# yifita/iso-points

Hardware: AMD Instinct MI355X
Metric: Mpoints/s full iso-point cycle (project+resample+splat), 1M pts (higher is better)
Workload: dtype f32-class (split-fp16 operands, 2^-22: hidden-layer products from two fp16 parts per f32 operand under exact power-of-two scales, 3 fp16-MFMA passes, f32 accumulate; everything else f32)

## Files before the change

iso_points_amd/csrc/bricks.hip:

```cpp
#include <type_traits>
#include "bricks.h"

#pragma clang fp contract(off)

constexpr int kScan1MaxWords = 2048;
BrickWs bricks_carve(void* ws, int64_t n_max) {
  BrickWs w;
  if (n_max < 1) n_max = 1;
  w.nb_cap = bricks_nb_cap(n_max);
  w.G = BK_CPB * (int64_t)w.nb_cap * w.nb_cap * w.nb_cap + 1;
  auto al = [](int64_t b) { return (b + 255) / 256 * 256; };
  char* p = (char*)ws;
  int64_t o = 0;
  w.hdr = (BrickHdr*)(p + o); o += al(sizeof(BrickHdr));
  w.counters = (int32_t*)(p + o); o += al(4 * kCounterInts);
  w.scan1 = (unsigned*)(p + o); o += al(4 * kScan1MaxWords);
  w.cnt = (int32_t*)(p + o); o += al(4 * w.G);
  w.off = (int32_t*)(p + o); o += al(4 * w.G);
  w.slot = (int32_t*)(p + o); o += al(4 * n_max);
  w.rec0 = (float4*)(p + o); o += al(16 * n_max);
  w.rec1 = (float4*)(p + o); o += al(16 * n_max);
  w.list = (int32_t*)(p + o); o += al(4 * (w.G < n_max ? w.G : n_max));
  w.tail = (int32_t*)(p + o); o += al(4 * 8 * n_max);
  w.scan_ws_bytes = iso_prefix_sum_workspace_bytes(w.G, 1) + 4 * (kScan1MaxWords + (w.G + 1023) / 1024);
// ... 984 lines not shown
__device__ __forceinline__ float wave_merge3(const Top3<KMAX>& best, int K, Emit&& emit) {
  int head = 0;
  float kth = FLT_MAX;
  for (int k = 0; k < K; ++k) {
    float hd = FLT_MAX;
    int hi = 0x7fffffff, ha = 0;
#pragma unroll
    for (int j = 0; j < KMAX; ++j) if (j == head) { hd = best.d[j]; hi = best.id[j]; ha = best.at[j]; }
    float md = hd;
    int mi = hi, ma = ha;
#pragma unroll
    for (int o = 32; o > 0; o >>= 1) {
      const float od = __shfl_xor(md, o);
      const int oi = __shfl_xor(mi, o), oa = __shfl_xor(ma, o);
      if (pair_lt(od, oi, md, mi)) { md = od; mi = oi; ma = oa; }
    }
    if (hd == md && hi == mi && md < FLT_MAX) ++head;
    if (k == K - 1) kth = md;
    emit(k, md, mi, ma);
  }
  return kth;
}

template <int KMAX>
__global__ __launch_bounds__(64) void k_brick_resample_tail(
    const BrickHdr* __restrict__ hp, const int32_t* __restrict__ off, const float4* __restrict__ rec0,
    const float4* __restrict__ rec1, const float* __restrict__ pts, int K, float* __restrict__ out,
    int64_t* __restrict__ idx_out, float* __restrict__ d2_out, const int32_t* __restrict__ tail,
    const int32_t* __restrict__ counters) {
  const BrickHdr h = *hp;
  const int lane = threadIdx.x;
  const int count = counters[1];
  const float B = 4.0f * h.f;
  const int rho_max = max(h.nb[0], max(h.nb[1], h.nb[2]));
  for (int w = blockIdx.x; w < count; w += gridDim.x) {
    const int row = tail[w];
    const float qx = pts[(int64_t)row * 3], qy = pts[(int64_t)row * 3 + 1], qz = pts[(int64_t)row * 3 + 2];
    const int qbx = bk_fine(qx, h.mn[0], h.inv_f, h.nf[0]) >> 2;
    const int qby = bk_fine(qy, h.mn[1], h.inv_f, h.nf[1]) >> 2;
    const int qbz = bk_fine(qz, h.mn[2], h.inv_f, h.nf[2]) >> 2;
    Top3<KMAX> best;
    best.init();
    float wd = FLT_MAX;
    int wi = 0x7fffffff;
    int found = 0;
    const WalkGeo geo = {qx, qy, qz, h.mn[0], h.mn[1], h.mn[2], B};
    float kth_seen = FLT_MAX;
    auto far2 = [&]() {
      float m = wd;
#pragma unroll
      for (int o = 32; o > 0; o >>= 1) m = fminf(m, __shfl_xor(m, o));
      return fminf(h.r2, fminf(m, kth_seen));
    };
    for (int rho = 0; rho <= rho_max; ++rho) {
      bk_walk_ring(rho, qbx, qby, qbz, h.nb[0], h.nb[1], h.nb[2], off, lane, geo, [&](int i) { return rec0[i]; },
                   [&](int i, const float4& c) {
        const float d2 = bk_d2(qx, qy, qz, c.x, c.y, c.z);
        if (d2 < h.r2) {
          if (found < KMAX) ++found;
          const int ci = __float_as_int(c.w);
          if (pair_lt(d2, ci, wd, wi)) {
            best.push(d2, ci, i, K);
#pragma unroll
            for (int j = 0; j < KMAX; ++j) if (j == K - 1) { wd = best.d[j]; wi = best.id[j]; }
          }
        }
      }, far2, far2);
      if (rho >= 1) {
        const float gg = (float)rho * B * 0.999f;
        if (gg >= h.r) break;
        int tot = found;
#pragma unroll
        for (int o = 32; o > 0; o >>= 1) tot += __shfl_xor(tot, o);
        if (tot >= K) {
          const float kth = wave_merge3<KMAX>(best, K, [](int, float, int, int) {});
          kth_seen = fminf(kth_seen, kth);
          if (kth < FLT_MAX && kth <= gg * gg) break;
        }
      }
    }
    Repulse R;
    R.px = qx; R.py = qy; R.pz = qz; R.inv_sigma = h.inv_sigma;
    const float kthf = wave_merge3<KMAX>(best, K, [&](int k, float md, int mi, int ma) {
      if (k == 0) return;
      if (md < FLT_MAX) {
        const float4 c = rec0[ma];
        const float4 u = rec1[ma];
        R.add(c.x, c.y, c.z, u.x, u.y, u.z);
      }
      if (idx_out && lane == 0) {
        idx_out[(int64_t)row * (K - 1) + k - 1] = md < FLT_MAX ? (int64_t)mi : (int64_t)-1;
        if (d2_out) d2_out[(int64_t)row * (K - 1) + k - 1] = md < FLT_MAX ? md : -1.0f;
      }
    });
    if (lane == 0) {
      R.finish(out + (int64_t)row * 3);
      const float need = kthf < FLT_MAX ? sqrtf(kthf) : h.r;
      if (qx - need < h.x_lo || qx + need >= h.x_hi) atomicAdd(const_cast<int32_t*>(&counters[6]), 1);
    }
  }
}

__global__ __launch_bounds__(256) void k_view_mask(const float* __restrict__ pts, const float* __restrict__ nrm,
                                                   const float* __restrict__ views, int n_views, int64_t n,
                                                   float znear, float zfar, int backface,
                                                   int32_t* __restrict__ mask, int32_t* __restrict__ view_count) {
  __shared__ int s_cnt[8];
  if (threadIdx.x < 8) s_cnt[threadIdx.x] = 0;
  __syncthreads();
  int local[8] = {0, 0, 0, 0, 0, 0, 0, 0};
  for (int64_t i = (int64_t)blockIdx.x * blockDim.x + threadIdx.x; i < n; i += (int64_t)gridDim.x * blockDim.x) {
    const float x = pts[i * 3], y = pts[i * 3 + 1], z = pts[i * 3 + 2];
    float nx = 0.f, ny = 0.f, nz = 0.f;
    if (backface) { nx = nrm[i * 3]; ny = nrm[i * 3 + 1]; nz = nrm[i * 3 + 2]; }
    int m = 0;
#pragma unroll
    for (int v = 0; v < 8; ++v) {
      if (v < n_views) {
        const float* V = views + v * 16;
        const float zv = ((x * V[2] + y * V[6]) + z * V[10]) + V[14];
// ... 197 lines not shown
  int pool_buf = 0;
  for (int w = blockIdx.x; w < count; w += gridDim.x) {
    const int row = tail[w] >> 3, v = tail[w] & 7;
    if (v >= n_views || !((mask[row] >> v) & 1)) continue;
    const float qx = pts[(int64_t)row * 3], qy = pts[(int64_t)row * 3 + 1], qz = pts[(int64_t)row * 3 + 2];
    const int qbx = bk_fine(qx, h.mn[0], h.inv_f, h.nf[0]) >> 2;
    const int qby = bk_fine(qy, h.mn[1], h.inv_f, h.nf[1]) >> 2;
    const int qbz = bk_fine(qz, h.mn[2], h.inv_f, h.nf[2]) >> 2;
    const bool small_cloud = view_total[v] < 7;
    TopF<7> best;
    best.init();
    float m7[7];
    const WalkGeo geo = {qx, qy, qz, h.mn[0], h.mn[1], h.mn[2], B};
    float kth_seen = FLT_MAX;
    bool sat = false;
    bool sat_any = false;
    bool sat_all = false;
    auto far2 = [&]() {
      float m = best.d[6];
#pragma unroll
      for (int o = 32; o > 0; o >>= 1) m = fminf(m, __shfl_xor(m, o));
      sat_any = sat_any || __any(sat);
      return fminf(sat_any ? kHSat : h.r2, fminf(m, kth_seen));
    };
    auto far2_all = [&]() { return fminf(sat_all ? kHSat : h.r2, kth_seen); };
    auto pool = [&]() {
      wave_merge_f7(best, m7);
      sat_any = sat_any || __any(sat);
      if (lane < 8) {
        float mine = m7[0];
#pragma unroll
        for (int k = 1; k < 7; ++k) mine = lane == k ? m7[k] : mine;
        s_m7[pool_buf][wave][lane] = lane == 7 ? (sat_any ? 1.f : 0.f) : mine;
      }
      __syncthreads();
      TopF<7> all;
      all.init();
      if (lane < 7 * kTailWaves) all.push(s_m7[pool_buf][lane / 7][lane % 7]);
      wave_merge_f7(all, m7);
#pragma unroll
      for (int k = 0; k < kTailWaves; ++k) sat_any = sat_any || s_m7[pool_buf][k][7] != 0.f;
      sat_all = sat_any;
      pool_buf ^= 1;
    };
    auto fetch = [&](int i) { float4 c = rec0[i]; c.w = rec1[i].w; return c; };
    auto visit = [&](int, const float4& c) {
      if (!((__float_as_int(c.w) >> v) & 1)) return;
      const float d2 = bk_d2(qx, qy, qz, c.x, c.y, c.z);
      if (d2 < kHSat) { if (d2 < h.r2) best.push(d2); }
      else if (d2 < h.r2) sat = true;
    };
    int rho_r = 1;
    while (rho_r < rho_max && (float)rho_r * B * 0.999f < h.r) ++rho_r;
    for (int rho = 0; rho <= min(1, rho_max); ++rho) {
      bk_walk_ring(rho, qbx, qby, qbz, h.nb[0], h.nb[1], h.nb[2], off, lane, geo, fetch, visit, far2_all, far2, wave, kTailWaves);
      if (rho >= 1) {
        const float gg = (float)rho * B * 0.999f;
        if (gg >= h.r) { rho_r = 1; break; }
        pool();
        kth_seen = fminf(kth_seen, m7[6]);
        if (m7[6] < FLT_MAX && m7[6] <= gg * gg) { rho_r = 1; break; }
        if (sat_any && kHSat <= gg * gg) { rho_r = 1; break; }
      }
    }
    if (rho_r > 1)
      bk_walk_shell(1, rho_r, qbx, qby, qbz, h.nb[0], h.nb[1], h.nb[2], off, lane, geo, fetch, visit, far2_all, far2, wave, kTailWaves);
    pool();
    if (threadIdx.x == 0) {
      const bool saturated = m7[6] == FLT_MAX && sat_any && !small_cloud;
      h_out[(int64_t)v * h.n_own + row] = saturated ? 0.01f : h_from_list(m7, small_cloud);
      const float need = m7[6] < FLT_MAX ? sqrtf(m7[6]) : (sat_any ? fminf(sqrtf(kHSat), h.r) : h.r);
      if (!small_cloud && (qx - need < h.x_lo || qx + need >= h.x_hi)) atomicAdd(const_cast<int32_t*>(&counters[6]), 1);
    }
  }
}

__device__ __forceinline__ void wave_append(bool take, int32_t* counter, int cap, int& slot) {
  const int lane = threadIdx.x & 63;
  const unsigned long long bal = __ballot(take);
  int base = 0;
  if (lane == 0 && bal) base = atomicAdd(counter, __popcll(bal));
  base = __shfl(base, 0);
  slot = take ? base + __popcll(bal & ((1ull << lane) - 1ull)) : -1;
  if (slot >= cap) slot = -1;
}

__global__ __launch_bounds__(256) void k_halo_export(const float* __restrict__ pts, const float* __restrict__ nrm,
                                                     const int32_t* __restrict__ payload, int64_t n_own,
                                                     const BrickHdr* __restrict__ hp, const float* __restrict__ ranges,
                                                     int world, int rank, int halo, float4* __restrict__ out, int cap) {
  const BrickHdr h = *hp;
  __shared__ int s_app[17];
  int32_t* counter = reinterpret_cast<int32_t*>(out);
  const int64_t span = (int64_t)gridDim.x * 1024;
  for (int64_t i0 = (int64_t)blockIdx.x * 1024; i0 < n_own; i0 += span) {
    bool take[4];
#pragma unroll
    for (int q = 0; q < 4; ++q) {
      const int64_t i = i0 + q * 256 + threadIdx.x;
      take[q] = false;
      if (i < n_own) {
        const int fx = bk_fine(pts[i * 3], h.mn[0], h.inv_f, h.nf[0]);
        for (int k = 0; k < world; ++k) {
          if (k == rank) continue;
          const int lo = bk_fine(ranges[k * 8], h.mn[0], h.inv_f, h.nf[0]) - halo;
          const int hi = bk_fine(ranges[k * 8 + 4], h.mn[0], h.inv_f, h.nf[0]) + halo;
          take[q] = take[q] || (fx >= lo && fx <= hi);
        }
      }
    }
    int slot[4];
    iso_block_append4(take, counter, s_app, slot);
#pragma unroll
    for (int q = 0; q < 4; ++q) {
      if (slot[q] >= 0 && slot[q] < cap) {
// ... 351 lines not shown
```

iso_points_amd/csrc/siren.hip:

```cpp
#include <stdlib.h>
#include "siren_common.h"
#include "iso_newton.h"
#include "mlp_common.h"

namespace {

__global__ void k_siren_pack(const float* __restrict__ raw, float* __restrict__ packed,
                             int H, int L) {
  const int64_t total = off_hidden(H, L);
  const int64_t HH = (int64_t)H * H;
  const int NT = H / 16;
  for (int64_t o = (int64_t)blockIdx.x * blockDim.x + threadIdx.x; o < total;
       o += (int64_t)gridDim.x * blockDim.x) {
    float v = 0.f;
    if (o < off_wl(H)) {
      int64_t k = o;
      int c = (int)(k & 3);
      int e = (int)((k >> 2) % (H / 4));
      int g = (int)((k >> 2) / (H / 4));
      int f = 16 * (e >> 2) + 4 * g + (e & 3);
      v = (c < 3) ? raw[f * 3 + c] : raw[(int64_t)H * 3 + f];
    } else if (o < off_bl(H)) {
      int64_t k = o - off_wl(H);
      int e = (int)(k % (H / 4));
      int g = (int)(k / (H / 4));
      int f = 16 * (e >> 2) + 4 * g + (e & 3);
      const int64_t raw_wl = (int64_t)H * 4 + (int64_t)L * (HH + H);
      v = raw[raw_wl + f];
    } else if (o < off_hidden(H, 0)) {
      const int64_t raw_wl = (int64_t)H * 4 + (int64_t)L * (HH + H);
      v = (o == off_bl(H)) ? raw[raw_wl + H] : 0.f;
    } else {
      int64_t k = o - off_hidden(H, 0);
      const int64_t per = H + 2 * HH;
      int l = (int)(k / per);
      int64_t w = k % per;
      const float* Wl = raw + (int64_t)H * 4 + (int64_t)l * (HH + H);
      const float* bl = Wl + HH;
      if (w < H) {
        v = bl[w];
      } else {
        w -= H;
        bool bwd = w >= HH;
        if (bwd) w -= HH;
        int i = (int)(w & 3);
        int lane = (int)((w >> 2) & 63);
        int t = (int)((w >> 8) % NT);
        int q = (int)((w >> 8) / NT);
        int a = 16 * t + (lane & 15);
        int b = 16 * q + 4 * (lane >> 4) + i;
        v = bwd ? Wl[(int64_t)b * H + a]
                : Wl[(int64_t)a * H + b];
      }
    }
    packed[o] = v;
  }
}

#define ISO_GEMM_FWD(img, bias) gemm_pass<NT, true>(img, bias, hL, wbuf, acc, lane, g)
#define ISO_GEMM_BWD(img) gemm_pass<NT, false>(img, nullptr, hL, wbuf, acc, lane, g)

template <int NT, bool CODED>
__global__ __launch_bounds__(256, 2) void k_siren_step(typename SirenArgsOf<CODED>::type a) {
  constexpr int H = NT * 16;
  extern __shared__ __attribute__((aligned(16))) float smem[];
  const int tid = threadIdx.x;
  const int wave = tid >> 6, lane = tid & 63;
  const int g = lane >> 4, j = lane & 15;
  float* hL = smem + wave * (NT * 256);
  float* wbuf = smem + 4 * NT * 256;
  const float* W0img = a.packed + off_w0(H);
  const float* WLimg = a.packed + off_wl(H);
  const float bL = a.packed[off_bl(H)];
  float* stash = a.stash + ((int64_t)blockIdx.x * 4 + wave) * (int64_t)(a.L + 1) * NT * 256;

  const int64_t count = a.count_in ? (int64_t)(*a.count_in) : a.n;
  const int64_t n_tiles = (count + 63) / 64;
  for (int64_t tile = blockIdx.x; tile < n_tiles; tile += gridDim.x) {
    const int64_t slot = tile * 64 + wave * 16 + j;
    const bool valid = slot < count;
    int64_t idx = -1;
    float px = 0.f, py = 0.f, pz = 0.f;
    int row = 0;
    if (valid) {
      idx = a.idx_in ? (int64_t)a.idx_in[slot] : slot;
      px = a.pts[idx * 3]; py = a.pts[idx * 3 + 1]; pz = a.pts[idx * 3 + 2];
      if constexpr (CODED) row = a.code_of ? a.code_of[idx] : 0;
    }
    const f32x4* cb = nullptr;
    if constexpr (CODED) cb = reinterpret_cast<const f32x4*>(a.code_bias + (int64_t)row * H) + g;
    (void)cb;
    float f = 0.f;
    const bool top0 = (a.L == 0);
    for (int e4 = 0; e4 < NT; ++e4) {
      f32x4 h4, s4;
      f32x4 b4 = {0.f, 0.f, 0.f, 0.f};
      if constexpr (CODED) b4 = cb[4 * e4];
#pragma unroll
      for (int i = 0; i < 4; ++i) {
        const f32x4 w = reinterpret_cast<const f32x4*>(W0img)[g * (H / 4) + e4 * 4 + i];
        float z;
        if constexpr (CODED) z = ((w.x * px + w.y * py) + w.z * pz) + b4[i];
        else z = ((w.x * px + w.y * py) + w.z * pz) + w.w;
        float s, c;
        iso_sincos(a.w0 * z, s, c);
        h4[i] = s;
        s4[i] = a.w0 * c;
      }
      if (top0) {
        const f32x4 w4 = reinterpret_cast<const f32x4*>(WLimg)[g * NT + e4];
// ... 114 lines not shown

bool siren_shape_ok(int H, int L) {
  return (H == 64 || H == 128 || H == 256) && L >= 0 && L <= 8;
}

int g_gemm_mode = -1;
int gemm_mode() {
  if (g_gemm_mode < 0) {
    const char* e = getenv("ISO_SIREN_GEMM");
    g_gemm_mode = (e && (!strcmp(e, "f32") || !strcmp(e, "0"))) ? 0 : 1;
  }
  return g_gemm_mode;
}
bool use_x3(int H, int L) { return gemm_mode() == 1 && siren_x3_supported(H, L); }

int64_t stash_floats_any(int H, int L) {
  int64_t a = stash_floats(H, L);
  int64_t b = siren_x3_supported(H, L) ? siren_x3_stash_floats(H, L) : 0;
  return a > b ? a : b;
}

int run_step(const SirenCodedArgs& a, int H, int64_t n, hipStream_t s) {
  if (use_x3(H, a.L)) return siren_x3_launch(a, H, n, s);
  int64_t tiles = (n + 63) / 64;
  int blocks = (int)(tiles < kSirenBlocks ? tiles : kSirenBlocks);
  return a.code_bias ? dispatch_step<true>(a, H, blocks, s) : dispatch_step<false>(a, H, blocks, s);
}

}

extern "C" int64_t iso_siren_raw_floats(int hidden, int n_hidden) {
  int64_t H = hidden;
  return H * 3 + H + (int64_t)n_hidden * (H * H + H) + H + 1;
}

extern "C" int64_t iso_siren_packed_floats(int hidden, int n_hidden) {
  return siren_packed_total(hidden, n_hidden);
}

extern "C" int iso_siren_set_gemm_mode(int mode) {
  ISO_REQUIRE(mode == 0 || mode == 1, ISO_ERR_INVALID, "iso_siren_set_gemm_mode: mode must be 0 (f32 MFMA) or 1 (split fp16)");
  g_gemm_mode = mode;
  return ISO_OK;
}

extern "C" int iso_siren_get_gemm_mode(void) { return gemm_mode(); }

extern "C" int iso_siren_pack_weights(const float* raw, float* packed, int hidden,
                                      int n_hidden, void* stream) {
  ISO_REQUIRE(siren_shape_ok(hidden, n_hidden), ISO_ERR_UNSUPPORTED,
              "iso_siren_pack_weights: hidden must be 64/128/256 and 0<=n_hidden<=8 (got %d, %d)",
              hidden, n_hidden);
  ISO_REQUIRE(raw && packed, ISO_ERR_INVALID, "iso_siren_pack_weights: null pointer");
  int64_t total = off_hidden(hidden, n_hidden);
  hipLaunchKernelGGL(k_siren_pack, dim3(iso_stream_grid(total, 256)), dim3(256), 0,
                     (hipStream_t)stream, raw, packed, hidden, n_hidden);
  if (hidden % 32 == 0) siren_x3_pack(raw, packed, hidden, n_hidden, (hipStream_t)stream);
  ISO_CHECK_LAUNCH("iso_siren_pack_weights");
  return ISO_OK;
}

static int64_t tail_cap_of(int64_t n) {
  const int64_t blocks = siren_x3_tail_blocks(), tiles = (n + 31) / 32;
  return ((tiles + blocks - 1) / blocks + 1) * 32;
}
static int64_t tail_ints(int64_t n) { return siren_x3_tail_blocks() * (2 * tail_cap_of(n) + 2); }

constexpr int kTileCtrInts = 128;
extern "C" int64_t iso_project_siren_workspace_bytes(int64_t n, int hidden, int n_hidden) {
  if (n < 0) n = 0;
  return stash_floats_any(hidden, n_hidden) * 4 + 2 * n * 4 + tail_ints(n) * 4 + (64 + kTileCtrInts) * 4 + 64;
}

extern "C" int64_t iso_project_siren_counts_offset(int64_t n, int hidden, int n_hidden) {
  if (n < 0) n = 0;
  return stash_floats_any(hidden, n_hidden) * 4 + 2 * n * 4 + tail_ints(n) * 4;
}

static int g_siren_dyn_tiles = -1;
static bool siren_dynamic_tiles_enabled() {
  return g_siren_dyn_tiles != 0;
}
extern "C" int iso_siren_set_drawn_tiles(int on) {
  ISO_REQUIRE(on >= -1 && on <= 1, ISO_ERR_INVALID, "iso_siren_set_drawn_tiles: -1 (default), 0 or 1");
  g_siren_dyn_tiles = on;
  return ISO_OK;
}

static int run_step_split(SirenCodedArgs a, int hidden, int64_t n, hipStream_t s) {
  if (hidden == 256 && !a.fwd_only && use_x3(hidden, a.L)) {
    a.split = 3;
    return run_step(a, hidden, n, s);
  }
  a.split = 0;
  a.tile_ctr = nullptr;
  return run_step(a, hidden, n, s);
}

static int g_tail_from = -1;
static int siren_tail_from(int max_iters) {
  if (g_tail_from == 0) return max_iters + 1;
  if (g_tail_from > 0) return g_tail_from;
  return max_iters >= 6 ? 4 : 2;
}
extern "C" int iso_siren_step_launches(int hidden, int n_hidden, int max_iters) {
  if (max_iters < 0) return 0;
  const bool can_tail = hidden == 256 && use_x3(hidden, n_hidden);
  const int from = can_tail ? siren_tail_from(max_iters) : max_iters + 1;
  return from <= max_iters && from > 0 ? from + 1 : max_iters + 1;
}
// ... 236 lines not shown
```

iso_points_amd/csrc/siren_common.h:

```cpp
#pragma once
#include "iso_common.h"

struct SirenArgs {
  float* pts;
  float* normals;
  uint8_t* mask;
  float* sdf_out;
  float* grad_out;
  const int32_t* idx_in;
  const int32_t* count_in;
  int32_t* idx_out;
  int32_t* count_out;
  const float* packed;
  float* stash;
  int64_t n;
  int L;
  float w0, wh, tol;
  int do_move;
  int eval_only;
  const float* dirs = nullptr;
  float alpha = 1.f, bound = 0.f, tol_valid = 0.f;
  int fwd_only = 0;
  int64_t cnt_lo = -1, cnt_hi = INT64_MAX;
  int small_tiles = 0;
  int split = 0;
  int big_blocks = 0;
  int32_t* tail_lists = nullptr;
  int32_t* tail_counts = nullptr;
  int32_t* iter_counts = nullptr;
  int tail_cap = 0, it_first = 0, it_last = 0;
  int32_t* tile_ctr = nullptr;
  int draw_first = 0;
  int ps_guard = 0;
};

struct SirenCodedArgs : SirenArgs {
  const float* code_bias = nullptr;
  const int32_t* code_of = nullptr;
};
template <bool CODED> struct SirenArgsOf { using type = SirenArgs; };
template <> struct SirenArgsOf<true> { using type = SirenCodedArgs; };

__host__ __device__ inline int64_t siren_split_point(int64_t count) {
  const int64_t big = 256 * 96, small = 256 * 32;
  const int64_t full = count / big * big, rem = count - full;
  if (rem == 0) return count;
  return (rem + small - 1) / small <= 2 ? full : count;
}

__host__ __device__ inline int64_t off_w0(int H) { (void)H; return 0; }
__host__ __device__ inline int64_t off_wl(int H) { return 4 * (int64_t)H; }
__host__ __device__ inline int64_t off_bl(int H) { return 5 * (int64_t)H; }
__host__ __device__ inline int64_t off_hidden(int H, int l) {
  return 5 * (int64_t)H + 4 + (int64_t)l * ((int64_t)H + 2 * (int64_t)H * H);
}

__host__ __device__ inline int x3_feat(int s, int kappa) {
  return 32 * (s >> 1) + 16 * (s & 1) + 8 * ((kappa & 7) >> 2) + 4 * (kappa >> 3) + (kappa & 3);
}
__host__ __device__ inline int64_t x3_base(int H, int L) { return off_hidden(H, L); }
__host__ __device__ inline int64_t x3_off_w0(int H, int L) { return x3_base(H, L); }
__host__ __device__ inline int64_t x3_off_wl(int H, int L) { return x3_base(H, L) + 4 * (int64_t)H; }
__host__ __device__ inline int64_t x3_off_layer(int H, int L, int l) {
  return x3_base(H, L) + 5 * (int64_t)H + (int64_t)l * (int64_t)H;
}
constexpr int kX16Header = 24;
__host__ __device__ inline int64_t x16_base(int H, int L) { return x3_off_layer(H, L, L); }
__host__ __device__ inline int64_t x16_off_layer(int H, int L, int l) { return x16_base(H, L) + kX16Header + (int64_t)l * H * H; }
__host__ __device__ inline int64_t x16_off_bw(int H, int L, int l) { return x16_off_layer(H, L, L) + (int64_t)l * H * H; }
__host__ __device__ inline int64_t siren_packed_total(int H, int L) { return x16_off_bw(H, L, L); }

bool siren_x3_supported(int H, int L);
int64_t siren_x3_stash_floats(int H, int L);
void siren_x3_pack(const float* raw, float* packed, int H, int L, hipStream_t s);
int siren_x3_launch(const SirenCodedArgs& a, int H, int64_t n_upper, hipStream_t s);
int siren_x3_tail_blocks();
int siren_x3_launch_tail(const SirenCodedArgs& a, int H, hipStream_t s);
constexpr int64_t kPsMinList = 3 * 256 * 128;
__host__ __device__ inline bool siren_ps_takes(int64_t count, int L, const float* hdr , float wh) {
  if (count < kPsMinList) return false;
  float r = 0.f;
  for (int l = 0; l < L; ++l) r = hdr[17 + l] > r ? hdr[17 + l] : r;
  return (wh * r) * 1.01f < 1.0e4f;
}
```

iso_points_amd/csrc/siren_x3.hip:

```cpp
#include <stdlib.h>
#include <type_traits>
#include "siren_common.h"
#include "iso_newton.h"
#include "mlp_common.h"

#include "mfma_split.h"

constexpr int kAD = 3;

namespace {

__device__ __forceinline__ void x3_sin_wcos8(float w_in, float w, const float (&z)[8], float (&s)[8], float (&c)[8]) {
  iso_sin_wcos8(w_in, w, z, s, c);
}


__global__ void k_siren_pack_x3(const float* __restrict__ raw, float* __restrict__ packed, int H, int L) {
  const int64_t base = x3_base(H, L), total = x16_base(H, L);
  const int64_t HH = (int64_t)H * H;
  const float* b0 = raw + (int64_t)H * 3;
  const float* WL = raw + (int64_t)H * 4 + (int64_t)L * (HH + H);
  for (int64_t o = base + (int64_t)blockIdx.x * blockDim.x + threadIdx.x; o < total;
       o += (int64_t)gridDim.x * blockDim.x) {
    const int64_t rel = o - base;
    auto feat_of = [](int64_t ko) { return x3_feat((int)(ko >> 4), 8 * (int)((ko >> 3) & 1) + (int)(ko & 7)); };
    if (rel < 4 * (int64_t)H) {
      const int f = feat_of(rel >> 2), c = (int)(rel & 3);
      packed[o] = (c < 3) ? raw[f * 3 + c] : b0[f];
    } else if (rel < 5 * (int64_t)H) {
      packed[o] = WL[feat_of(rel - 4 * (int64_t)H)];
    } else {
      const int64_t r2 = rel - 5 * (int64_t)H;
      const int l = (int)(r2 / H);
      const float* Wl = raw + (int64_t)H * 4 + (int64_t)l * (HH + H);
      packed[o] = Wl[HH + feat_of(r2 % H)];
    }
  }
}

__global__ void k_siren_wscale(const float* __restrict__ raw, float* __restrict__ packed, int H, int L) {
  __shared__ float s_m[256];
  const int l = blockIdx.x;
  const int64_t HH = (int64_t)H * H;
  const float* Wl = raw + (int64_t)H * 4 + (int64_t)l * (HH + H);
  float m = 0.f, cs = 0.f;
  for (int f = threadIdx.x; f < H; f += 256) {
    float t = 0.f;
#pragma unroll 32
    for (int k = 0; k < H; ++k) {
      const float a = fabsf(Wl[(int64_t)k * H + f]);
      m = (a == a && a > m) ? a : m;
      t += a;
    }
    cs = fmaxf(cs, t);
  }
  s_m[threadIdx.x] = m;
  __syncthreads();
  for (int o = 128; o > 0; o >>= 1) {
    if ((int)threadIdx.x < o) s_m[threadIdx.x] = fmaxf(s_m[threadIdx.x], s_m[threadIdx.x + o]);
    __syncthreads();
  }
  if (threadIdx.x == 0) {
    float mx = s_m[0];
    int e = 0;
    float sc = 1.0f;
    if (mx > 0.f && mx < 3.0e38f) {
      (void)frexpf(mx, &e);
      int k = 10 - e;
      k = k > 100 ? 100 : (k < -100 ? -100 : k);
      sc = ldexpf(1.0f, k);
    }
    packed[x16_base(H, L) + l] = sc;
  }
  __syncthreads();
  s_m[threadIdx.x] = cs;
  __syncthreads();
  for (int o = 128; o > 0; o >>= 1) {
    if ((int)threadIdx.x < o) s_m[threadIdx.x] = fmaxf(s_m[threadIdx.x], s_m[threadIdx.x + o]);
    __syncthreads();
  }
  if (threadIdx.x == 0) packed[x16_base(H, L) + 8 + l] = s_m[0];
  if (l == 0) {
    __syncthreads();
    const float* WLh = raw + (int64_t)H * 4 + (int64_t)L * (HH + H);
    float mh = 0.f;
    for (int f = threadIdx.x; f < H; f += 256) mh = fmaxf(mh, fabsf(WLh[f]));
    s_m[threadIdx.x] = mh;
    __syncthreads();
    for (int o = 128; o > 0; o >>= 1) {
      if ((int)threadIdx.x < o) s_m[threadIdx.x] = fmaxf(s_m[threadIdx.x], s_m[threadIdx.x + o]);
      __syncthreads();
    }
    if (threadIdx.x == 0) packed[x16_base(H, L) + 16] = s_m[0];
  }
}

__global__ void k_siren_pack_f16(const float* __restrict__ raw, float* __restrict__ packed, int H, int L) {
  const int64_t HH = (int64_t)H * H;
  const int NTO = H / 32;
  const int64_t total = 2 * (int64_t)L * HH;
  for (int64_t o = (int64_t)blockIdx.x * blockDim.x + threadIdx.x; o < total; o += (int64_t)gridDim.x * blockDim.x) {
    const bool bwd = o >= (int64_t)L * HH;
    const int l = (int)((o / HH) % L);
    const int64_t q = o % HH;
    const float* Wl = raw + (int64_t)H * 4 + (int64_t)l * (HH + H);
    const float sc = packed[x16_base(H, L) + l];
    const int d = (int)(q & 3), lane = (int)((q >> 2) & 63);
    const int64_t blk = q >> 8;
    const int part = (int)(blk & 1);
    const int To = (int)((blk >> 1) % NTO), s = (int)(blk / (2 * NTO));
    const int fo = 32 * To + (lane & 31);
    f32x2 v;
#pragma unroll
    for (int u = 0; u < 2; ++u) {
      const int fi = x3_feat(s, 8 * (lane >> 5) + 2 * d + u);
      v[u] = (bwd ? Wl[(int64_t)fi * H + fo] : Wl[(int64_t)fo * H + fi]) * sc;
    }
    const f16x2 h = __builtin_convertvector(v, f16x2);
    const f16x2 lo = __builtin_convertvector(v - __builtin_convertvector(h, f32x2), f16x2);
    reinterpret_cast<unsigned*>(packed + x16_off_layer(H, L, 0))[o] =
        part == 0 ? __builtin_bit_cast(unsigned, h) : __builtin_bit_cast(unsigned, lo);
  }
}

template <int H, int NW, int NB>
struct X3Shape {
  static constexpr int NS = H / 16;
  static constexpr int NTO = H / 32;
  static constexpr int TW = NTO / NW;
  static constexpr int SL = 2 * TW;
  static constexpr int NG = SL * NB;
  static constexpr int P = 32 * NB;
  static constexpr size_t kActBytes = (size_t)NS * NB * kAP * 1024;
  static constexpr size_t kRedBytes = (size_t)NW * P * 16;
  static constexpr size_t kPtsBytes = (size_t)P * 16;
  static constexpr int kLdsGroupsFit = (int)((163840 - (kActBytes + kRedBytes + kPtsBytes)) / ((size_t)NW * 2048));
  static constexpr int LG = kLdsGroupsFit < NG ? kLdsGroupsFit : NG;
  static constexpr size_t kLds = kActBytes + kRedBytes + kPtsBytes + (size_t)NW * LG * 2048;
  static constexpr int64_t kStashPerWg(int L) { return (int64_t)NW * (L > 1 ? L : 1) * NG * 512; }
  static_assert(NTO % NW == 0 && TW >= 1, "features must split evenly over the waves");
};

template <int H>
__device__ __forceinline__ void x3_code_bias8(const float* table, int row, int s, int h, float (&b)[8]) {
  const f32x4* t = reinterpret_cast<const f32x4*>(table + (int64_t)row * H + 16 * s + 4 * h);
  const f32x4 lo = t[0], hi = t[2];
#pragma unroll
  for (int e = 0; e < 4; ++e) { b[e] = lo[e]; b[4 + e] = hi[e]; }
}

template <int H, int NW, int NB, bool FWD, bool CODED>
__device__ __forceinline__ void x3_step_body(const typename SirenArgsOf<CODED>::type& a, const int bid, const int nblk,
                                             const int sid) {
  using S = X3Shape<H, NW, NB>;
  constexpr int NS = S::NS, NTO = S::NTO, TW = S::TW, SL = S::SL, NG = S::NG, P = S::P;
  extern __shared__ __attribute__((aligned(16))) unsigned char smem_raw[];
  u32x4* act = reinterpret_cast<u32x4*>(smem_raw);
  f32x4* red = reinterpret_cast<f32x4*>(smem_raw + S::kActBytes);
  f32x4* ptl = reinterpret_cast<f32x4*>(smem_raw + S::kActBytes + S::kRedBytes);
  constexpr int LG = S::LG;
  const int tid = threadIdx.x;
  const int w = __builtin_amdgcn_readfirstlane(tid >> 6);
  const int lane = tid & 63, h = lane >> 5, j = lane & 31;
  u32x4* own = act + (size_t)(SL * w) * NB * kAP * 64 + lane;
  u32x4* park = own + (size_t)(kAP - 2) * NG * 64;
  constexpr bool IL = (NW == 8);
  const int L = a.L;
  const float* X = a.packed + x3_base(H, L);
  const f32x4* W0u = reinterpret_cast<const f32x4*>(X) + SL * w * 16;
  const float* WLu = X + 4 * H + SL * w * 16;
  const int h8 = h * 8;
  const float bL = a.packed[off_bl(H)];
  f32x4* stash = reinterpret_cast<f32x4*>(a.stash) +
                 ((int64_t)sid * NW + w) * (int64_t)(L > 1 ? L : 1) * NG * 128;
// ... 442 lines not shown
}

template <int H, int NW, int NB, int MINB, bool FWD, bool CODED>
int launch_x3(const typename SirenArgsOf<CODED>::type& a, int64_t n_upper, hipStream_t s) {
  using S = X3Shape<H, NW, NB>;
  static bool attr_done = false;
  if (!attr_done) {
    (void)hipFuncSetAttribute(reinterpret_cast<const void*>(&k_siren_step_x3<H, NW, NB, MINB, FWD, CODED>),
                              hipFuncAttributeMaxDynamicSharedMemorySize, (int)S::kLds);
    attr_done = true;
  }
  const int64_t tiles = (n_upper + S::P - 1) / S::P;
  const int64_t cap = 256 * MINB;
  const int blocks = (int)(tiles < cap ? (tiles < 1 ? 1 : tiles) : cap);
  hipLaunchKernelGGL((k_siren_step_x3<H, NW, NB, MINB, FWD, CODED>), dim3(blocks), dim3(64 * NW), S::kLds, s, a);
  return 0;
}

template <int H, int NW, int NB, int MINB, bool CODED>
int launch_x3_both(typename SirenArgsOf<CODED>::type a, int64_t n_upper, hipStream_t s) {
  using SB = X3Shape<H, NW, NB>;
  using SS = X3Shape<H, NW, 1>;
  constexpr size_t lds = SB::kLds > SS::kLds ? SB::kLds : SS::kLds;
  static bool attr_done = false;
  if (!attr_done) {
    (void)hipFuncSetAttribute(reinterpret_cast<const void*>(&k_siren_step_x3_both<H, NW, NB, MINB, CODED>),
                              hipFuncAttributeMaxDynamicSharedMemorySize, (int)lds);
    attr_done = true;
  }
  const int64_t cap = 256 * MINB;
  const int64_t tb = (n_upper + SB::P - 1) / SB::P, ts = (n_upper + SS::P - 1) / SS::P;
  a.big_blocks = (int)(tb < cap ? (tb < 1 ? 1 : tb) : cap);
  const int small_blocks = (int)(ts < cap ? (ts < 1 ? 1 : ts) : cap);
  hipLaunchKernelGGL((k_siren_step_x3_both<H, NW, NB, MINB, CODED>), dim3(a.big_blocks + small_blocks), dim3(64 * NW), lds, s, a);
  return 0;
}

}

constexpr int kNW256 = 8;
constexpr int kMinB256 = 1;
constexpr int kNB256 = 3;
constexpr int kMinB128 = 1;
bool siren_x3_supported(int H, int L) { return (H == 256 || H == 128) && L >= 1 && L <= 8; }

int64_t siren_x3_stash_floats(int H, int L) {
  if (H == 256) {
    return 256 * kMinB256 * (X3Shape<256, kNW256, kNB256>::kStashPerWg(L) + X3Shape<256, kNW256, 1>::kStashPerWg(L));
  }
  if (H == 128) return 256 * kMinB128 * X3Shape<128, 4, 3>::kStashPerWg(L);
  return 0;
}

void siren_x3_pack(const float* raw, float* packed, int H, int L, hipStream_t s) {
  const int64_t words = x16_base(H, L) - x3_base(H, L);
  hipLaunchKernelGGL(k_siren_pack_x3, dim3(iso_stream_grid(words, 256)), dim3(256), 0, s, raw, packed, H, L);
  if (L > 0) {
    hipLaunchKernelGGL(k_siren_wscale, dim3(L), dim3(256), 0, s, raw, packed, H, L);
    hipLaunchKernelGGL(k_siren_pack_f16, dim3(iso_stream_grid(2 * (int64_t)L * H * H, 256)), dim3(256), 0, s, raw, packed, H, L);
  }
}

int siren_x3_tail_blocks() { return 256 * kMinB256; }

template <bool CODED>
static int launch_tail(const typename SirenArgsOf<CODED>::type& a, hipStream_t s) {
  using SS = X3Shape<256, kNW256, 1>;
  static bool attr_done = false;
  if (!attr_done) {
    (void)hipFuncSetAttribute(reinterpret_cast<const void*>(&k_siren_tail_x3<256, kNW256, kMinB256, CODED>),
                              hipFuncAttributeMaxDynamicSharedMemorySize, (int)SS::kLds);
    attr_done = true;
  }
  hipLaunchKernelGGL((k_siren_tail_x3<256, kNW256, kMinB256, CODED>), dim3(siren_x3_tail_blocks()), dim3(64 * kNW256), SS::kLds, s, a);
  return 0;
}

int siren_x3_launch_tail(const SirenCodedArgs& a, int H, hipStream_t s) {
  if (H != 256) return -1;
  return a.code_bias ? launch_tail<true>(a, s) : launch_tail<false>(a, s);
}

template <bool CODED>
static int launch_any(const typename SirenArgsOf<CODED>::type& a, int H, int64_t n_upper, hipStream_t s) {
  if (a.split == 3 && H == 256 && !a.fwd_only) return launch_x3_both<256, kNW256, kNB256, kMinB256, CODED>(a, n_upper, s);
  if (a.fwd_only) {
    if (H == 256) return launch_x3<256, kNW256, kNB256, kMinB256, true, CODED>(a, n_upper, s);
    if (H == 128) return launch_x3<128, 4, 3, kMinB128, true, CODED>(a, n_upper, s);
  }
  if constexpr (!CODED) {
    if (H == 256) return launch_x3<256, kNW256, kNB256, kMinB256, false, false>(a, n_upper, s);
  }
  if (H == 128) return launch_x3<128, 4, 3, kMinB128, false, CODED>(a, n_upper, s);
  return -1;
}

int siren_x3_launch(const SirenCodedArgs& a, int H, int64_t n_upper, hipStream_t s) {
  return a.code_bias ? launch_any<true>(a, H, n_upper, s) : launch_any<false>(a, H, n_upper, s);
}
```

Before: 74.08.

## Fuse SIREN weight packing into one kernel and walk inner brick shell at once

The four weight-packing launches (f32 section, x3 k-order, per-layer scale, f16 split) are merged into one kernel with role-partitioned workgroups. Each f16 workgroup recomputes the layer absmax scale itself, so it no longer depends on a separate scale kernel. The header reduction is vectorised and uses a shared reduction helper. In the brick kNN and tail searches, rings 0 and 1 are now visited in a single shell walk instead of two ring walks, which cuts per-ring overhead and the early-exit checks after ring 0. The cost is redundant absmax passes over each layer's weights (one per f16 workgroup) and a different visit order in the neighbour search.

```diff
diff --git a/iso_points_amd/csrc/bricks.hip b/iso_points_amd/csrc/bricks.hip
--- a/iso_points_amd/csrc/bricks.hip
+++ b/iso_points_amd/csrc/bricks.hip
@@ -1060,20 +1060,22 @@
       for (int o = 32; o > 0; o >>= 1) m = fminf(m, __shfl_xor(m, o));
       return fminf(h.r2, fminf(m, kth_seen));
     };
-    for (int rho = 0; rho <= rho_max; ++rho) {
-      bk_walk_ring(rho, qbx, qby, qbz, h.nb[0], h.nb[1], h.nb[2], off, lane, geo, [&](int i) { return rec0[i]; },
-                   [&](int i, const float4& c) {
-        const float d2 = bk_d2(qx, qy, qz, c.x, c.y, c.z);
-        if (d2 < h.r2) {
-          if (found < KMAX) ++found;
-          const int ci = __float_as_int(c.w);
-          if (pair_lt(d2, ci, wd, wi)) {
-            best.push(d2, ci, i, K);
-#pragma unroll
-            for (int j = 0; j < KMAX; ++j) if (j == K - 1) { wd = best.d[j]; wi = best.id[j]; }
-          }
+    auto fetch = [&](int i) { return rec0[i]; };
+    auto visit = [&](int i, const float4& c) {
+      const float d2 = bk_d2(qx, qy, qz, c.x, c.y, c.z);
+      if (d2 < h.r2) {
+        if (found < KMAX) ++found;
+        const int ci = __float_as_int(c.w);
+        if (pair_lt(d2, ci, wd, wi)) {
+          best.push(d2, ci, i, K);
+#pragma unroll
+          for (int j = 0; j < KMAX; ++j) if (j == K - 1) { wd = best.d[j]; wi = best.id[j]; }
         }
-      }, far2, far2);
+      }
+    };
+    for (int rho = min(1, rho_max); rho <= rho_max; ++rho) {
+      if (rho <= 1) bk_walk_shell(-1, rho, qbx, qby, qbz, h.nb[0], h.nb[1], h.nb[2], off, lane, geo, fetch, visit, far2, far2);
+      else bk_walk_ring(rho, qbx, qby, qbz, h.nb[0], h.nb[1], h.nb[2], off, lane, geo, fetch, visit, far2, far2);
       if (rho >= 1) {
         const float gg = (float)rho * B * 0.999f;
         if (gg >= h.r) break;
@@ -1377,15 +1379,16 @@
     };
     int rho_r = 1;
     while (rho_r < rho_max && (float)rho_r * B * 0.999f < h.r) ++rho_r;
-    for (int rho = 0; rho <= min(1, rho_max); ++rho) {
-      bk_walk_ring(rho, qbx, qby, qbz, h.nb[0], h.nb[1], h.nb[2], off, lane, geo, fetch, visit, far2_all, far2, wave, kTailWaves);
-      if (rho >= 1) {
-        const float gg = (float)rho * B * 0.999f;
-        if (gg >= h.r) { rho_r = 1; break; }
+    const int rho1 = min(1, rho_max);
+    bk_walk_shell(-1, rho1, qbx, qby, qbz, h.nb[0], h.nb[1], h.nb[2], off, lane, geo, fetch, visit, far2_all, far2, wave, kTailWaves);
+    if (rho1 >= 1) {
+      const float gg = (float)rho1 * B * 0.999f;
+      if (gg >= h.r) rho_r = 1;
+      else {
         pool();
         kth_seen = fminf(kth_seen, m7[6]);
-        if (m7[6] < FLT_MAX && m7[6] <= gg * gg) { rho_r = 1; break; }
-        if (sat_any && kHSat <= gg * gg) { rho_r = 1; break; }
+        if (m7[6] < FLT_MAX && m7[6] <= gg * gg) rho_r = 1;
+        else if (sat_any && kHSat <= gg * gg) rho_r = 1;
       }
     }
     if (rho_r > 1)
diff --git a/iso_points_amd/csrc/siren.hip b/iso_points_amd/csrc/siren.hip
--- a/iso_points_amd/csrc/siren.hip
+++ b/iso_points_amd/csrc/siren.hip
@@ -4,58 +4,6 @@
 #include "mlp_common.h"
 
 namespace {
-
-__global__ void k_siren_pack(const float* __restrict__ raw, float* __restrict__ packed,
-                             int H, int L) {
-  const int64_t total = off_hidden(H, L);
-  const int64_t HH = (int64_t)H * H;
-  const int NT = H / 16;
-  for (int64_t o = (int64_t)blockIdx.x * blockDim.x + threadIdx.x; o < total;
-       o += (int64_t)gridDim.x * blockDim.x) {
-    float v = 0.f;
-    if (o < off_wl(H)) {
-      int64_t k = o;
-      int c = (int)(k & 3);
-      int e = (int)((k >> 2) % (H / 4));
-      int g = (int)((k >> 2) / (H / 4));
-      int f = 16 * (e >> 2) + 4 * g + (e & 3);
-      v = (c < 3) ? raw[f * 3 + c] : raw[(int64_t)H * 3 + f];
-    } else if (o < off_bl(H)) {
-      int64_t k = o - off_wl(H);
-      int e = (int)(k % (H / 4));
-      int g = (int)(k / (H / 4));
-      int f = 16 * (e >> 2) + 4 * g + (e & 3);
-      const int64_t raw_wl = (int64_t)H * 4 + (int64_t)L * (HH + H);
-      v = raw[raw_wl + f];
-    } else if (o < off_hidden(H, 0)) {
-      const int64_t raw_wl = (int64_t)H * 4 + (int64_t)L * (HH + H);
-      v = (o == off_bl(H)) ? raw[raw_wl + H] : 0.f;
-    } else {
-      int64_t k = o - off_hidden(H, 0);
-      const int64_t per = H + 2 * HH;
-      int l = (int)(k / per);
-      int64_t w = k % per;
-      const float* Wl = raw + (int64_t)H * 4 + (int64_t)l * (HH + H);
-      const float* bl = Wl + HH;
-      if (w < H) {
-        v = bl[w];
-      } else {
-        w -= H;
-        bool bwd = w >= HH;
-        if (bwd) w -= HH;
-        int i = (int)(w & 3);
-        int lane = (int)((w >> 2) & 63);
-        int t = (int)((w >> 8) % NT);
-        int q = (int)((w >> 8) / NT);
-        int a = 16 * t + (lane & 15);
-        int b = 16 * q + 4 * (lane >> 4) + i;
-        v = bwd ? Wl[(int64_t)b * H + a]
-                : Wl[(int64_t)a * H + b];
-      }
-    }
-    packed[o] = v;
-  }
-}
 
 #define ISO_GEMM_FWD(img, bias) gemm_pass<NT, true>(img, bias, hL, wbuf, acc, lane, g)
 #define ISO_GEMM_BWD(img) gemm_pass<NT, false>(img, nullptr, hL, wbuf, acc, lane, g)
@@ -276,10 +224,7 @@
               "iso_siren_pack_weights: hidden must be 64/128/256 and 0<=n_hidden<=8 (got %d, %d)",
               hidden, n_hidden);
   ISO_REQUIRE(raw && packed, ISO_ERR_INVALID, "iso_siren_pack_weights: null pointer");
-  int64_t total = off_hidden(hidden, n_hidden);
-  hipLaunchKernelGGL(k_siren_pack, dim3(iso_stream_grid(total, 256)), dim3(256), 0,
-                     (hipStream_t)stream, raw, packed, hidden, n_hidden);
-  if (hidden % 32 == 0) siren_x3_pack(raw, packed, hidden, n_hidden, (hipStream_t)stream);
+  siren_pack_all(raw, packed, hidden, n_hidden, (hipStream_t)stream);
   ISO_CHECK_LAUNCH("iso_siren_pack_weights");
   return ISO_OK;
 }
diff --git a/iso_points_amd/csrc/siren_common.h b/iso_points_amd/csrc/siren_common.h
--- a/iso_points_amd/csrc/siren_common.h
+++ b/iso_points_amd/csrc/siren_common.h
@@ -55,6 +55,49 @@
   return 5 * (int64_t)H + 4 + (int64_t)l * ((int64_t)H + 2 * (int64_t)H * H);
 }
 
+__device__ inline float siren_f32_section_word(const float* __restrict__ raw, int H, int L, int64_t o) {
+  const int64_t HH = (int64_t)H * H;
+  const int NT = H / 16;
+  if (o < off_wl(H)) {
+    int64_t k = o;
+    int c = (int)(k & 3);
+    int e = (int)((k >> 2) % (H / 4));
+    int g = (int)((k >> 2) / (H / 4));
+    int f = 16 * (e >> 2) + 4 * g + (e & 3);
+    return (c < 3) ? raw[f * 3 + c] : raw[(int64_t)H * 3 + f];
+  }
+  if (o < off_bl(H)) {
+    int64_t k = o - off_wl(H);
+    int e = (int)(k % (H / 4));
+    int g = (int)(k / (H / 4));
+    int f = 16 * (e >> 2) + 4 * g + (e & 3);
+    const int64_t raw_wl = (int64_t)H * 4 + (int64_t)L * (HH + H);
+    return raw[raw_wl + f];
+  }
+  if (o < off_hidden(H, 0)) {
+    const int64_t raw_wl = (int64_t)H * 4 + (int64_t)L * (HH + H);
+    return (o == off_bl(H)) ? raw[raw_wl + H] : 0.f;
+  }
+  int64_t k = o - off_hidden(H, 0);
+  const int64_t per = H + 2 * HH;
+  int l = (int)(k / per);
+  int64_t w = k % per;
+  const float* Wl = raw + (int64_t)H * 4 + (int64_t)l * (HH + H);
+  const float* bl = Wl + HH;
+  if (w < H) return bl[w];
+  w -= H;
+  bool bwd = w >= HH;
+  if (bwd) w -= HH;
+  int i = (int)(w & 3);
+  int lane = (int)((w >> 2) & 63);
+  int t = (int)((w >> 8) % NT);
+  int q = (int)((w >> 8) / NT);
+  int a = 16 * t + (lane & 15);
+  int b = 16 * q + 4 * (lane >> 4) + i;
+  return bwd ? Wl[(int64_t)b * H + a]
+             : Wl[(int64_t)a * H + b];
+}
+
 __host__ __device__ inline int x3_feat(int s, int kappa) {
   return 32 * (s >> 1) + 16 * (s & 1) + 8 * ((kappa & 7) >> 2) + 4 * (kappa >> 3) + (kappa & 3);
 }
@@ -72,7 +115,7 @@
 
 bool siren_x3_supported(int H, int L);
 int64_t siren_x3_stash_floats(int H, int L);
-void siren_x3_pack(const float* raw, float* packed, int H, int L, hipStream_t s);
+void siren_pack_all(const float* raw, float* packed, int H, int L, hipStream_t s);
 int siren_x3_launch(const SirenCodedArgs& a, int H, int64_t n_upper, hipStream_t s);
 int siren_x3_tail_blocks();
 int siren_x3_launch_tail(const SirenCodedArgs& a, int H, hipStream_t s);
diff --git a/iso_points_amd/csrc/siren_x3.hip b/iso_points_amd/csrc/siren_x3.hip
--- a/iso_points_amd/csrc/siren_x3.hip
+++ b/iso_points_amd/csrc/siren_x3.hip
@@ -15,111 +15,134 @@
 }
 
 
-__global__ void k_siren_pack_x3(const float* __restrict__ raw, float* __restrict__ packed, int H, int L) {
-  const int64_t base = x3_base(H, L), total = x16_base(H, L);
-  const int64_t HH = (int64_t)H * H;
-  const float* b0 = raw + (int64_t)H * 3;
-  const float* WL = raw + (int64_t)H * 4 + (int64_t)L * (HH + H);
-  for (int64_t o = base + (int64_t)blockIdx.x * blockDim.x + threadIdx.x; o < total;
-       o += (int64_t)gridDim.x * blockDim.x) {
-    const int64_t rel = o - base;
-    auto feat_of = [](int64_t ko) { return x3_feat((int)(ko >> 4), 8 * (int)((ko >> 3) & 1) + (int)(ko & 7)); };
-    if (rel < 4 * (int64_t)H) {
-      const int f = feat_of(rel >> 2), c = (int)(rel & 3);
-      packed[o] = (c < 3) ? raw[f * 3 + c] : b0[f];
-    } else if (rel < 5 * (int64_t)H) {
-      packed[o] = WL[feat_of(rel - 4 * (int64_t)H)];
-    } else {
-      const int64_t r2 = rel - 5 * (int64_t)H;
-      const int l = (int)(r2 / H);
-      const float* Wl = raw + (int64_t)H * 4 + (int64_t)l * (HH + H);
-      packed[o] = Wl[HH + feat_of(r2 % H)];
-    }
-  }
-}
-
-__global__ void k_siren_wscale(const float* __restrict__ raw, float* __restrict__ packed, int H, int L) {
-  __shared__ float s_m[256];
-  const int l = blockIdx.x;
+constexpr int kPackWgs = 32;
+
+__device__ __forceinline__ float x3_wscale_of(float mx) {
+  int e = 0;
+  float sc = 1.0f;
+  if (mx > 0.f && mx < 3.0e38f) {
+    (void)frexpf(mx, &e);
+    int k = 10 - e;
+    k = k > 100 ? 100 : (k < -100 ? -100 : k);
+    sc = ldexpf(1.0f, k);
+  }
+  return sc;
+}
+
+__device__ __forceinline__ float x3_wg_max(float m, float* s_m) {
+  __syncthreads();
+  s_m[threadIdx.x] = m;
+  __syncthreads();
+  for (int o = 128; o > 0; o >>= 1) {
+    if ((int)threadIdx.x < o) s_m[threadIdx.x] = fmaxf(s_m[threadIdx.x], s_m[threadIdx.x + o]);
+    __syncthreads();
+  }
+  return s_m[0];
+}
+
+__device__ __forceinline__ float x3_absmax(float m, float v) { return fmaxf(m, fabsf(v)); }
+
+__device__ __forceinline__ void x3_pack_header(const float* __restrict__ raw, float* __restrict__ packed, int H, int L,
+                                               int l, float* s_m) {
   const int64_t HH = (int64_t)H * H;
   const float* Wl = raw + (int64_t)H * 4 + (int64_t)l * (HH + H);
   float m = 0.f, cs = 0.f;
   for (int f = threadIdx.x; f < H; f += 256) {
     float t = 0.f;
-#pragma unroll 32
-    for (int k = 0; k < H; ++k) {
-      const float a = fabsf(Wl[(int64_t)k * H + f]);
-      m = (a == a && a > m) ? a : m;
-      t += a;
+    for (int k0 = 0; k0 < H; k0 += 64) {
+      float v[64];
+#pragma unroll
+      for (int k = 0; k < 64; ++k) v[k] = Wl[(int64_t)(k0 + k) * H + f];
+#pragma unroll
+      for (int k = 0; k < 64; ++k) {
+        m = x3_absmax(m, v[k]);
+        t += fabsf(v[k]);
+      }
     }
     cs = fmaxf(cs, t);
   }
-  s_m[threadIdx.x] = m;
-  __syncthreads();
-  for (int o = 128; o > 0; o >>= 1) {
-    if ((int)threadIdx.x < o) s_m[threadIdx.x] = fmaxf(s_m[threadIdx.x], s_m[threadIdx.x + o]);
-    __syncthreads();
-  }
-  if (threadIdx.x == 0) {
-    float mx = s_m[0];
-    int e = 0;
-    float sc = 1.0f;
-    if (mx > 0.f && mx < 3.0e38f) {
-      (void)frexpf(mx, &e);
-      int k = 10 - e;
-      k = k > 100 ? 100 : (k < -100 ? -100 : k);
-      sc = ldexpf(1.0f, k);
-    }
-    packed[x16_base(H, L) + l] = sc;
-  }
-  __syncthreads();
-  s_m[threadIdx.x] = cs;
-  __syncthreads();
-  for (int o = 128; o > 0; o >>= 1) {
-    if ((int)threadIdx.x < o) s_m[threadIdx.x] = fmaxf(s_m[threadIdx.x], s_m[threadIdx.x + o]);
-    __syncthreads();
-  }
-  if (threadIdx.x == 0) packed[x16_base(H, L) + 8 + l] = s_m[0];
+  const float mx = x3_wg_max(m, s_m);
+  if (threadIdx.x == 0) packed[x16_base(H, L) + l] = x3_wscale_of(mx);
+  const float c = x3_wg_max(cs, s_m);
+  if (threadIdx.x == 0) packed[x16_base(H, L) + 8 + l] = c;
   if (l == 0) {
-    __syncthreads();
     const float* WLh = raw + (int64_t)H * 4 + (int64_t)L * (HH + H);
     float mh = 0.f;
     for (int f = threadIdx.x; f < H; f += 256) mh = fmaxf(mh, fabsf(WLh[f]));
-    s_m[threadIdx.x] = mh;
-    __syncthreads();
-    for (int o = 128; o > 0; o >>= 1) {
-      if ((int)threadIdx.x < o) s_m[threadIdx.x] = fmaxf(s_m[threadIdx.x], s_m[threadIdx.x + o]);
-      __syncthreads();
-    }
-    if (threadIdx.x == 0) packed[x16_base(H, L) + 16] = s_m[0];
-  }
-}
-
-__global__ void k_siren_pack_f16(const float* __restrict__ raw, float* __restrict__ packed, int H, int L) {
-  const int64_t HH = (int64_t)H * H;
-  const int NTO = H / 32;
-  const int64_t total = 2 * (int64_t)L * HH;
-  for (int64_t o = (int64_t)blockIdx.x * blockDim.x + threadIdx.x; o < total; o += (int64_t)gridDim.x * blockDim.x) {
-    const bool bwd = o >= (int64_t)L * HH;
-    const int l = (int)((o / HH) % L);
-    const int64_t q = o % HH;
-    const float* Wl = raw + (int64_t)H * 4 + (int64_t)l * (HH + H);
-    const float sc = packed[x16_base(H, L) + l];
-    const int d = (int)(q & 3), lane = (int)((q >> 2) & 63);
-    const int64_t blk = q >> 8;
-    const int part = (int)(blk & 1);
-    const int To = (int)((blk >> 1) % NTO), s = (int)(blk / (2 * NTO));
+    mh = x3_wg_max(mh, s_m);
+    if (threadIdx.x == 0) packed[x16_base(H, L) + 16] = mh;
+  }
+}
+
+__device__ __forceinline__ void x3_pack_f16(const float* __restrict__ raw, float* __restrict__ packed, int H, int L,
+                                            int l, int part_wg, float* s_m) {
+  const int HH = H * H;
+  const int lgH = __ffs(H) - 1, lgT = lgH - 5;
+  const float* Wl = raw + (int64_t)H * 4 + (int64_t)l * ((int64_t)HH + H);
+  float m = 0.f;
+  if ((reinterpret_cast<uintptr_t>(Wl) & 15) == 0) {
+    const f32x4* W4 = reinterpret_cast<const f32x4*>(Wl);
+#pragma unroll 16
+    for (int i = threadIdx.x; i < HH / 4; i += 256) {
+      const f32x4 v = W4[i];
+      m = x3_absmax(x3_absmax(x3_absmax(x3_absmax(m, v[0]), v[1]), v[2]), v[3]);
+    }
+  } else {
+#pragma unroll 16
+    for (int i = threadIdx.x; i < HH; i += 256) m = x3_absmax(m, Wl[i]);
+  }
+  const float sc = x3_wscale_of(x3_wg_max(m, s_m));
+  unsigned* img = reinterpret_cast<unsigned*>(packed + x16_off_layer(H, L, 0));
+#pragma unroll 8
+  for (int i = part_wg * 256 + (int)threadIdx.x; i < 2 * HH; i += kPackWgs * 256) {
+    const bool bwd = i >= HH;
+    const int q = bwd ? i - HH : i;
+    const int64_t o = ((int64_t)(bwd ? L : 0) + l) * HH + q;
+    const int d = q & 3, lane = (q >> 2) & 63;
+    const int blk = q >> 8;
+    const int part = blk & 1;
+    const int To = (blk >> 1) & ((1 << lgT) - 1), s = blk >> (1 + lgT);
     const int fo = 32 * To + (lane & 31);
     f32x2 v;
 #pragma unroll
     for (int u = 0; u < 2; ++u) {
       const int fi = x3_feat(s, 8 * (lane >> 5) + 2 * d + u);
-      v[u] = (bwd ? Wl[(int64_t)fi * H + fo] : Wl[(int64_t)fo * H + fi]) * sc;
+      v[u] = (bwd ? Wl[(fi << lgH) + fo] : Wl[(fo << lgH) + fi]) * sc;
     }
     const f16x2 h = __builtin_convertvector(v, f16x2);
     const f16x2 lo = __builtin_convertvector(v - __builtin_convertvector(h, f32x2), f16x2);
-    reinterpret_cast<unsigned*>(packed + x16_off_layer(H, L, 0))[o] =
-        part == 0 ? __builtin_bit_cast(unsigned, h) : __builtin_bit_cast(unsigned, lo);
+    img[o] = part == 0 ? __builtin_bit_cast(unsigned, h) : __builtin_bit_cast(unsigned, lo);
+  }
+}
+
+__device__ __forceinline__ float x3_korder_word(const float* __restrict__ raw, int H, int L, int64_t o) {
+  const int64_t HH = (int64_t)H * H;
+  const float* b0 = raw + (int64_t)H * 3;
+  const float* WL = raw + (int64_t)H * 4 + (int64_t)L * (HH + H);
+  const int64_t rel = o - x3_base(H, L);
+  auto feat_of = [](int64_t ko) { return x3_feat((int)(ko >> 4), 8 * (int)((ko >> 3) & 1) + (int)(ko & 7)); };
+  if (rel < 4 * (int64_t)H) {
+    const int f = feat_of(rel >> 2), c = (int)(rel & 3);
+    return (c < 3) ? raw[f * 3 + c] : b0[f];
+  }
+  if (rel < 5 * (int64_t)H) return WL[feat_of(rel - 4 * (int64_t)H)];
+  const int64_t r2 = rel - 5 * (int64_t)H;
+  const int l = (int)(r2 / H);
+  const float* Wl = raw + (int64_t)H * 4 + (int64_t)l * (HH + H);
+  return Wl[HH + feat_of(r2 % H)];
+}
+
+__global__ __launch_bounds__(256) void k_siren_pack_all(const float* __restrict__ raw, float* __restrict__ packed, int H, int L) {
+  __shared__ float s_m[256];
+  const int b = blockIdx.x;
+  if (b < L) {
+    x3_pack_header(raw, packed, H, L, b, s_m);
+  } else if (b < L + kPackWgs * L) {
+    x3_pack_f16(raw, packed, H, L, (b - L) / kPackWgs, (b - L) % kPackWgs, s_m);
+  } else {
+    const int64_t o = (int64_t)(b - L - kPackWgs * L) * 256 + threadIdx.x;
+    if (o < x3_base(H, L)) packed[o] = siren_f32_section_word(raw, H, L, o);
+    else if (o < x16_base(H, L)) packed[o] = x3_korder_word(raw, H, L, o);
   }
 }
 
@@ -668,13 +691,10 @@
   return 0;
 }
 
-void siren_x3_pack(const float* raw, float* packed, int H, int L, hipStream_t s) {
-  const int64_t words = x16_base(H, L) - x3_base(H, L);
-  hipLaunchKernelGGL(k_siren_pack_x3, dim3(iso_stream_grid(words, 256)), dim3(256), 0, s, raw, packed, H, L);
-  if (L > 0) {
-    hipLaunchKernelGGL(k_siren_wscale, dim3(L), dim3(256), 0, s, raw, packed, H, L);
-    hipLaunchKernelGGL(k_siren_pack_f16, dim3(iso_stream_grid(2 * (int64_t)L * H * H, 256)), dim3(256), 0, s, raw, packed, H, L);
-  }
+void siren_pack_all(const float* raw, float* packed, int H, int L, hipStream_t s) {
+  const int64_t words = x16_base(H, L);
+  const int grid = L + kPackWgs * L + (int)((words + 255) / 256);
+  hipLaunchKernelGGL(k_siren_pack_all, dim3(grid), dim3(256), 0, s, raw, packed, H, L);
 }
 
 int siren_x3_tail_blocks() { return 256 * kMinB256; }
```

Result: no change. 74.23, median of 6 (+0.2%).
